# mackelab/poisson-gpfa

Measured on AMD Instinct MI355X. Metric: EM iterations/sec, higher is better.
Workload: dtype f64

## Files before the change

poisson-gpfa_amd/csrc/chol.h:

```cpp
#pragma once
#include "types.h"

namespace pgpfa {


__device__ __forceinline__ int potrf_lidx(int j, int r) { return j * NB - (j * (j - 1)) / 2 + (r - j); }

template <typename T>
struct PotrfLds {
  T L[NB * (NB + 1) / 2];
  T line[2][NB];
  T rd[2];
  T rowc[2][2][64];
  T colc[2][NB];
};

template <typename T>
__device__ __forceinline__ T pick8(const T* a, int k) {
  const T v01 = (k & 1) ? a[1] : a[0], v23 = (k & 1) ? a[3] : a[2];
  const T v45 = (k & 1) ? a[5] : a[4], v67 = (k & 1) ? a[7] : a[6];
  const T v03 = (k & 2) ? v23 : v01, v47 = (k & 2) ? v67 : v45;
  return (k & 4) ? v47 : v03;
}

template <int Q, typename T>
__device__ __forceinline__ void potrf_diag_chol_steps(T (&a)[32], PotrfLds<T>& S, int r, int cg, int pos_r,
                                                       int* __restrict__ info, long long slot, int k0) {
#pragma unroll 1
  for (int j = 32 * Q; j < 32 * Q + 32; ++j) {
    const bool own = (j & 3) == cg;
    T* buf = S.line[j & 1];
    if (own && r >= j) {
      const T v = pick8(&a[8 * Q], (j >> 2) - 8 * Q);
      buf[pos_r] = v;
      if (r == j) {
        T rd = rsqrt(v);
        if (!(v > (T)0)) {
          if (info[slot] == 0) info[slot] = k0 + j + 1;
          rd = (T)1;
        }
        S.rd[j & 1] = rd;
      }
    }
    __syncthreads();
    if (r >= j) {
      const T rd = S.rd[j & 1];
      const T lr = buf[pos_r] * rd;
      if (own) S.L[potrf_lidx(j, r)] = lr;
      const T nlr = -lr * rd;
      const T* bp = buf + cg * 32;
#pragma unroll
      for (int m = 8 * Q; m < 32; ++m) a[m] = fma(nlr, bp[m], a[m]);
    }
  }
}

template <int S, typename T>
__device__ __forceinline__ void potrf_diag_chol_steps2(T (&a)[4][8], PotrfLds<T>& L, int tr, int tc, int* __restrict__ info, long long slot, int k0) {
  typedef T v2 __attribute__((ext_vector_type(2)));
#pragma unroll 1
  for (int j = 16 * S; j < 16 * S + 16; ++j) {
    const int b = j & 1;
    if (tc == (j & 15)) {
      *reinterpret_cast<v2*>(&L.rowc[b][0][2 * tr]) = v2{a[0][S], a[1][S]};
      *reinterpret_cast<v2*>(&L.rowc[b][1][2 * tr]) = v2{a[2][S], a[3][S]};
#pragma unroll
      for (int i = 0; i < 4; ++i) L.colc[b][(tr & 15) * 8 + 2 * i + (tr >> 4)] = a[i][S];
      if (tr == (j & 31)) {
        const T v = (j >> 5) == 0 ? a[0][S] : (j >> 5) == 1 ? a[1][S] : (j >> 5) == 2 ? a[2][S] : a[3][S];
        T rd = rsqrt(v);
        if (!(v > (T)0)) {
          if (info[slot] == 0) info[slot] = k0 + j + 1;
          rd = (T)1;
        }
        L.rd[b] = rd;
      }
    }
    __syncthreads();
    const T rd = L.rd[b];
    const v2 r01 = *reinterpret_cast<const v2*>(&L.rowc[b][0][2 * tr]), r23 = *reinterpret_cast<const v2*>(&L.rowc[b][1][2 * tr]);
    T lr[4] = {r01.x * rd, r01.y * rd, r23.x * rd, r23.y * rd};
    if (tc == (j & 15)) {
#pragma unroll
      for (int i = 0; i < 4; ++i) {
        const int r = tr + 32 * i;
        if (r >= j) L.L[potrf_lidx(j, r)] = lr[i];
      }
    }
    T cv[8];
#pragma unroll
    for (int m = S & ~1; m < 8; m += 2) {
      const v2 c2 = *reinterpret_cast<const v2*>(&L.colc[b][8 * tc + m]);
      cv[m] = c2.x; cv[m + 1] = c2.y;
    }
#pragma unroll
    for (int i = 0; i < 4; ++i) {
      const T nlr = -lr[i] * rd;
#pragma unroll
      for (int m = S; m < 8; ++m) a[i][m] = fma(nlr, cv[m], a[i][m]);
    }
  }
}

template <typename T>
__device__ __forceinline__ void potrf_diag_inverse(PotrfLds<T>& S, int tid, int r, int cg) {
  const int Q = r >> 5, rl = r & 31;
  const T inv_lrr = (T)1 / S.L[potrf_lidx(r, r)];
  T t[8];
#pragma unroll
  for (int m = 0; m < 8; ++m) t[m] = (T)0;
#pragma unroll 1
  for (int il = 0; il < 32; ++il) {
    T* xrow = S.line[il & 1] + Q * 32 + cg * 8;
    if (rl == il) {
#pragma unroll
      for (int m = 0; m < 8; ++m) xrow[m] = t[m];
      if ((il & 3) == cg) xrow[il >> 2] = inv_lrr;
    }
    __syncthreads();
    if (rl > il) {
      const T lri = -S.L[potrf_lidx(32 * Q + il, r)] * inv_lrr;
#pragma unroll
      for (int m = 0; m < 8; ++m) t[m] = fma(lri, xrow[m], t[m]);
    }
  }
  __syncthreads();
#pragma unroll
  for (int m = 0; m < 8; ++m) {
    const int c = 32 * Q + cg + 4 * m;
    if (c < r) S.L[potrf_lidx(c, r)] = t[m];
  }
  if ((rl & 3) == cg) S.L[potrf_lidx(r, r)] = inv_lrr;
  __syncthreads();
  using V4 = typename GemmVec<T>::v4;
  const int lane = tid & 63, wave = tid >> 6, l15 = lane & 15, l4 = lane >> 4;
  auto lrow = [](int i) { return i * (NB - 1) - (i * (i - 1)) / 2; };
  auto xoff = [](int c) { return c * NB - (c * (c - 1)) / 2 - c; };
#pragma unroll 1
  for (int P = 1; P < 4; ++P) {
    const int ntile = 4 * P;
    V4 acc[2];
#pragma unroll
    for (int s2 = 0; s2 < 2; ++s2) {
      acc[s2] = V4{(T)0, (T)0, (T)0, (T)0};
      const int tile = wave + 8 * s2;
      if (tile < ntile) {
        const int rt = tile & 1, ct = tile >> 1;
        const int row = 32 * P + 16 * rt + l15, col = 16 * ct + l15;
        const int xo = xoff(col);
        for (int k0 = 16 * ct; k0 < 32 * P; k0 += 4) {
          const int k = k0 + l4;
          const T av = S.L[lrow(k) + row];
          const T bv = S.L[xo + k];
          acc[s2] = gemm_mfma16(av, (k >= col) ? bv : (T)0, acc[s2]);
        }
      }
    }
    __syncthreads();
#pragma unroll
    for (int s2 = 0; s2 < 2; ++s2) {
      const int tile = wave + 8 * s2;
      if (tile < ntile) {
        const int rt = tile & 1, ct = tile >> 1;
        const int xo = xoff(16 * ct + l15);
#pragma unroll
        for (int q = 0; q < 4; ++q) S.L[xo + 32 * P + 16 * rt + (sizeof(T) == 8 ? l4 + 4 * q : 4 * l4 + q)] = acc[s2][q];
      }
    }
    __syncthreads();
#pragma unroll
    for (int s2 = 0; s2 < 2; ++s2) {
      acc[s2] = V4{(T)0, (T)0, (T)0, (T)0};
      const int tile = wave + 8 * s2;
      if (tile < ntile) {
        const int rt = tile & 1, ct = tile >> 1;
        const int row = 32 * P + 16 * rt + l15;
        const int xo = xoff(16 * ct + l15);
        for (int k0 = 32 * P; k0 < 32 * P + 16 * (rt + 1); k0 += 4) {
          const int k = k0 + l4;
          const T av = S.L[lrow(k <= row ? k : row) + row];
          const T bv = S.L[xo + k];
          acc[s2] = gemm_mfma16((k <= row) ? -av : (T)0, bv, acc[s2]);
        }
      }
    }
    __syncthreads();
#pragma unroll
    for (int s2 = 0; s2 < 2; ++s2) {
      const int tile = wave + 8 * s2;
      if (tile < ntile) {
        const int rt = tile & 1, ct = tile >> 1;
        const int xo = xoff(16 * ct + l15);
#pragma unroll
        for (int q = 0; q < 4; ++q) S.L[xo + 32 * P + 16 * rt + (sizeof(T) == 8 ? l4 + 4 * q : 4 * l4 + q)] = acc[s2][q];
      }
    }
    __syncthreads();
  }
}

template <typename T, int PH = 3, int ALG = 2, typename TS = T>
__global__ __launch_bounds__(512) void potrf_diag_kernel_t(TS* __restrict__ H, long long sH, int ld, int k0,
                                                            TS* __restrict__ Dinv, long long sD,
                                                            const int* __restrict__ slots, int* __restrict__ info) {
  __shared__ __attribute__((aligned(16))) PotrfLds<T> S;
  const int tid = threadIdx.x;
  const int r = tid & (NB - 1);
  const int cg = tid >> 7;
  const int pos_r = (r & 3) * 32 + (r >> 2);
  const long long slot = slots ? slots[blockIdx.x] : blockIdx.x;
  TS* Hs = H + slot * sH + (size_t)k0 * ld + k0;
  TS* Ds = Dinv + slot * sD + (size_t)(k0 / NB) * NB * NB;

  if constexpr (ALG == 2) {
    const int tr = tid & 31, tc = tid >> 5;
    T a2[4][8];
#pragma unroll
    for (int i = 0; i < 4; ++i)
#pragma unroll
      for (int m = 0; m < 8; ++m) a2[i][m] = (T)Hs[(size_t)(tc + 16 * m) * ld + tr + 32 * i];
    if constexpr (PH & 1) {
      potrf_diag_chol_steps2<0>(a2, S, tr, tc, info, slot, k0);
      potrf_diag_chol_steps2<1>(a2, S, tr, tc, info, slot, k0);
      potrf_diag_chol_steps2<2>(a2, S, tr, tc, info, slot, k0);
      potrf_diag_chol_steps2<3>(a2, S, tr, tc, info, slot, k0);
      potrf_diag_chol_steps2<4>(a2, S, tr, tc, info, slot, k0);
      potrf_diag_chol_steps2<5>(a2, S, tr, tc, info, slot, k0);
      potrf_diag_chol_steps2<6>(a2, S, tr, tc, info, slot, k0);
      potrf_diag_chol_steps2<7>(a2, S, tr, tc, info, slot, k0);
    } else {
#pragma unroll
      for (int i = 0; i < 4; ++i)
#pragma unroll
        for (int m = 0; m < 8; ++m)
          if (tc + 16 * m <= tr + 32 * i) S.L[potrf_lidx(tc + 16 * m, tr + 32 * i)] = a2[i][m];
    }
  } else {
    T a[32];
#pragma unroll
    for (int m = 0; m < 32; ++m) a[m] = (T)Hs[(size_t)(cg + 4 * m) * ld + r];
    if constexpr (PH & 1) {
      potrf_diag_chol_steps<0>(a, S, r, cg, pos_r, info, slot, k0);
      potrf_diag_chol_steps<1>(a, S, r, cg, pos_r, info, slot, k0);
      potrf_diag_chol_steps<2>(a, S, r, cg, pos_r, info, slot, k0);
      potrf_diag_chol_steps<3>(a, S, r, cg, pos_r, info, slot, k0);
    } else {
#pragma unroll
      for (int m = 0; m < 32; ++m)
        if (cg + 4 * m <= r) S.L[potrf_lidx(cg + 4 * m, r)] = a[m];
    }
  }
  __syncthreads();
  for (int e = tid; e < NB * NB; e += 512) {
    const int rr = e & (NB - 1), cc = e >> 7;
    if (rr >= cc) Hs[(size_t)cc * ld + rr] = (TS)S.L[potrf_lidx(cc, rr)];
  }
  if constexpr (PH & 2) potrf_diag_inverse(S, tid, r, cg);
  for (int e = tid; e < NB * NB; e += 512) {
    const int rr = e & (NB - 1), cc = e >> 7;
    Ds[(size_t)cc * NB + rr] = (rr >= cc) ? (TS)S.L[potrf_lidx(cc, rr)] : (TS)0;
  }
}

template <typename T>
__global__ void diag_transpose_kernel_t(T* __restrict__ Mt, long long sM, int ld, int k0,
                                        const T* __restrict__ Dinv, long long sD, const int* __restrict__ slots) {
  const long long slot = slots ? slots[blockIdx.x] : blockIdx.x;
  k0 += blockIdx.y * NB;
  T* M = Mt + slot * sM + (size_t)k0 * ld + k0;
  const T* D = Dinv + slot * sD + (size_t)(k0 / NB) * NB * NB;
  __shared__ T tile[32][33];
  const int tx = threadIdx.x & 31, ty = threadIdx.x >> 5;
  for (int sub = 0; sub < 16; ++sub) {
    const int br = (sub & 3) * 32, bc = (sub >> 2) * 32;
    __syncthreads();
#pragma unroll
    for (int i = 0; i < 4; ++i) tile[ty + 8 * i][tx] = D[(br + ty + 8 * i) * NB + bc + tx];
    __syncthreads();
#pragma unroll
    for (int i = 0; i < 4; ++i) M[(size_t)(bc + ty + 8 * i) * ld + br + tx] = tile[tx][ty + 8 * i];
  }
}

inline __global__ __launch_bounds__(256) void chol_solve_kernel(const double* __restrict__ H, long long sH, int ld, int npad,
                                                          const double* __restrict__ Dinv, long long sD,
                                                          const double* __restrict__ G, double* __restrict__ V,
                                                          long long sV, const int* __restrict__ slots,
                                                          double* __restrict__ dec, double* __restrict__ smax, int n) {
  __shared__ double yk[NB];
  __shared__ double zk[NB];
  __shared__ double red[8];
  const int tid = threadIdx.x;
  const int lane = tid & 63, wave = tid >> 6;
  const long long slot = slots ? slots[blockIdx.x] : blockIdx.x;
  const double* L = H + slot * sH;
  const double* D = Dinv + slot * sD;
  const double* g = G + slot * sV;
  double* v = V + slot * sV;
  const int nblk = npad / NB;

  for (int i = tid; i < npad; i += 256) v[i] = (i < n) ? g[i] : 0.0;
  __syncthreads();
  for (int kb = 0; kb < nblk; ++kb) {
    const int k0 = kb * NB;
// ... 60 lines not shown
```

poisson-gpfa_amd/csrc/core.hip:

```cpp
#include "ctx.h"
#include "model.h"
#include "dual.h"
#include "thin.h"
#include "hook.h"
#include "plan.h"

using namespace pgpfa;

static_assert(plan::Dims{}.NB == NB && plan::Dims{}.WIDE_MAX == WIDE_MAX, "plan.h restates two constants of the kernel headers (workspace.hip includes none)");

thread_local std::string g_err;
thread_local unsigned long long g_fail_count = 0;

int fail(const char* fmt, ...) {
  char buf[1024];
  va_list ap;
  va_start(ap, fmt);
  vsnprintf(buf, sizeof(buf), fmt, ap);
  va_end(ap);
  g_err = buf;
  ++g_fail_count;
  return 1;
}

// ... 820 lines not shown
  };
  if (k == "newton_xtol") c->xtol = v;
  else if (k == "newton_max_iter") c->max_iter = (int)v;
  else if (k == "use_mfma") {
    const bool was = c->mfma;
    c->mfma = (v != 0.0);
    if (c->have_params && c->rank_gran != 16 && was != c->mfma)
      CHK(pgpfa_set_params(c, std::vector<double>(c->hC).data(), std::vector<double>(c->hd).data(), std::vector<double>(c->htau).data()));
  }
  else if (k == "cd_mfma") c->cd_mfma = (v != 0.0);
  else if (k == "cd_hess_mfma") c->cd_hess_mfma = (v != 0.0);
  else if (k == "cross_kernel") c->cross_kernel = (v != 0.0);
  else if (k == "cd_debug") c->cd_debug = (int)v;
  else if (k == "pcg_fused") c->pcg_fused = (int)v;
  else if (k == "pcg_w32") c->pcg_w32 = (v != 0.0);
  else if (k == "pcg_form") c->pcg_form = (int)v;
  else if (k == "pcg_vec32") c->pcg_vec32 = (int)v;
  else if (k == "pcg_rx32") c->pcg_rx32 = (int)v;
  else if (k == "pcg_adapt") c->pcg_adapt = (int)v;
  else if (k == "pcg_xcd") c->pcg_xcd = (int)v;
  else if (k == "mt_fill") c->mt_fill = (int)v;
  else if (k == "overlap_factors") c->overlap_factors = (int)v;
  else if (k == "mix_slot") c->mix_slot = (int)v;
  else if (k == "yt_mix") c->yt_mix = (v != 0.0);
  else if (k == "pivchol_pairs") c->pivchol_pairs = (v != 0.0);
  else if (k == "vsm_b4") c->vsm_b4 = (int)v;
  else if (k == "poisson_tiles") c->poisson_tiles = (int)v;
  else if (k == "yt_mix_dbg") c->yt_mix_dbg = (int)v;
  else if (k == "yt_mix_dma") c->yt_mix_dma = (v != 0.0);
  else if (k == "syrk_dbg") c->syrk_dbg = (int)v;
  else if (k == "syrk_tile") c->syrk_tile = (int)v;
  else if (k == "mix_wide") c->mix_wide = (int)v;
  else if (k == "thin_products") {
    const bool was = c->thin_products >= 2;
    c->thin_products = (int)v;
    if (c->have_params && c->rank_gran != 16 && was != (c->thin_products >= 2))
      CHK(pgpfa_set_params(c, std::vector<double>(c->hC).data(), std::vector<double>(c->hd).data(), std::vector<double>(c->htau).data()));
  }
  else if (k == "copy_kernels") c->copy_kernels = (v != 0.0);
  else if (k == "chord") c->chord = (v != 0.0);
  else if (k == "shared_pcg") c->shared_pcg = (v != 0.0);
  else if (k == "time_newton") c->time_newton = (v != 0.0);
  else if (k == "pcg_trace") c->pcg_trace = (v != 0.0);
  else if (k == "measure_mix") { c->measure_mix = (v != 0.0); c->info["last_eps_wt_norm"] = 0.0; c->info["last_eps_wt_rms"] = 0.0; }
  else if (k == "pcg_retire") c->pcg_retire = (v != 0.0);
  else if (k == "split_cov") c->split_cov = (v != 0.0);
  else if (k == "split_max_norm") c->split_max_norm = v;
  else if (k == "cov_mode") c->cov_mode = (int)v;
  else if (k == "lowrank_tol") {
    const bool changed = c->lr_tol != v;
    c->lr_tol = v;
    if (c->have_params && changed)
      CHK(pgpfa_set_params(c, std::vector<double>(c->hC).data(), std::vector<double>(c->hd).data(), std::vector<double>(c->htau).data()));
  }
  else if (k == "keep_trial_vsmgp") c->keep_trial_vsmgp = (v != 0.0);
  else if (k == "dual_lowrank") c->dual_lowrank = (v != 0.0);
  else if (k == "dual_f32") c->dual_f32 = (int)v;
  else if (k == "laplace_f32") { if (v != 0.0 && v != 1.0 && v != 2.0) return fail("laplace_f32 is 0, 1 or 2"); c->laplace_f32 = (int)v; }
  else if (k == "dual_masked") { if (v != 0.0 && v != 1.0) return fail("dual_masked is 0 or 1"); c->dual_masked = (int)v; }
  else if (k == "laplace_evidence") { if (v != 0.0 && v != 1.0) return fail("laplace_evidence is 0 or 1"); c->laplace_evidence = (int)v; }
  else if (k == "sample_chunk_trials") CHK(chunk_trials(&c->sample_chunk));
  else if (k == "interp_chunk_trials") CHK(chunk_trials(&c->interp_chunk));
  else if (k == "covat_chunk_trials") CHK(chunk_trials(&c->covat_chunk));
  else if (k == "velat_chunk_trials") CHK(chunk_trials(&c->velat_chunk));
  else if (k == "covat_block_times") { if (v < 0.0 || v != std::floor(v)) return fail("covat_block_times is a count of query times, or 0"); c->covat_block = (int)v; }
  else if (k == "func_chunk_trials") CHK(chunk_trials(&c->func_chunk));
  else if (k == "func_block_cols") {
    if (v < 0.0 || v != std::floor(v) || std::fmod(v, 16.0) != 0.0) return fail("func_block_cols is a count of functionals that is a multiple of 16, or 0");
    c->func_block = (int)v;
  }
  else if (k == "rates_chunk_trials") CHK(chunk_trials(&c->rates_chunk));
  else if (k == "counts_chunk_trials") CHK(chunk_trials(&c->counts_chunk));
  else if (k == "counts_nodes") { if (v < 8.0 || v > 64.0 || v != std::floor(v)) return fail("counts_nodes is a node count in 8 .. 64"); c->counts_Q = (int)v; }
  else if (k == "slab_row_align") c->slab_row_align = (v != 0.0);
  else if (k == "vsm_mfma") c->vsm_mfma = (v != 0.0);
  else if (k == "dual_gemm") c->dual_gemm = (v != 0.0);
  else if (k == "extrapolate_start") c->extrapolate = (v != 0.0);
  else if (k == "extrapolate_beta") c->extrapolate_beta = v;
  else if (k == "extrapolate_guard") c->extrapolate_guard = v;
  else if (k == "start_guard") c->start_guard = (v != 0.0);
  else if (k == "shared_min") c->shared_min = (int)v;
  else if (k == "pcg_inner") c->pcg_inner_max = std::max(1, (int)v);
  else if (k == "pcg_eta0") c->pcg_eta0 = v;
  else if (k == "splitk_target") c->splitk_target = std::max(1, (int)v);
  else if (k == "small_tile_below") c->small_tile_below = (int)v;
  else if (k == "f32_tile64") c->f32_tile64 = (int)v;
  else if (k == "splitk_below64") c->splitk_below64 = (int)v;
  else if (k == "pcg_outer_max") c->pcg_outer_max = (int)v;
  else if (k == "chord_xtol") c->chord_xtol = v;
  else if (k == "chord_rho") c->chord_rho = v;
  else if (k == "chord_max_step") c->chord_max_step = v;
  else if (k == "chord_max") c->chord_max = (int)v;
  else if (k == "chunk_trials") { if (c->B > 0) return fail("chunk_trials must be set before the first E-step"); c->chunk_opt = (int)v; }
  else if (k == "workspace_headroom") c->arena_headroom = std::max(1.0, v);
  else if (k == "rank_gran") { if (v != 4.0 && v != 8.0 && v != 16.0) return fail("rank_gran is 4, 8 or 16"); c->rank_gran = (int)v; if (c->have_params) CHK(pgpfa_set_params(c, std::vector<double>(c->hC).data(), std::vector<double>(c->hd).data(), std::vector<double>(c->htau).data())); }
  else if (k == "workspace_pool") { if (c->arena_cap > 0) return fail("workspace_pool must be set before the first E-step"); c->use_pool = (v != 0.0); }
  else if (k == "workspace_grow_budget_ms") c->grow_budget_ms = v;
  else if (k == "workspace_grow_floor_slots") c->grow_floor_slots = std::max(1, (int)v);
  else if (k == "workspace_granule_mb") c->vmm_granule = (size_t)std::max(2.0, v) << 20;
  else if (k == "workspace_vmm") { if (c->arena_cap > 0) return fail("workspace_vmm must be set before the first E-step"); c->vmm = (v != 0.0) ? 0 : -1; }
  else if (k == "eps_noise") {
    const bool changed = c->eps != v;
    c->eps = v;
    if (c->have_params && changed)
      CHK(pgpfa_set_params(c, std::vector<double>(c->hC).data(), std::vector<double>(c->hd).data(), std::vector<double>(c->htau).data()));
  }
  else if (k == "profile") {
    if (v != 0.0) {
      prof_collect(c);
      c->prof.ms.clear(); c->prof.flops.clear(); c->prof.count.clear(); c->prof.max_ms.clear(); c->prof.max_flops.clear(); c->prof.shapes.clear();
      HIPC(hipSetDevice(c->device));
      const size_t want = 2 * (256 + 64) + 2;
      while (c->prof.pool.size() < want) {
        hipEvent_t e;
        HIPC(hipEventCreate(&e));
        c->prof.pool.push_back(e);
        c->prof.idle.push_back(e);
      }
      for (int rep = 0; rep < 8; ++rep)
        for (hipEvent_t e : c->prof.idle) HIPC(hipEventRecord(e, c->st));
      HIPC(hipStreamSynchronize(c->st));
    }
    c->prof.on = (v != 0.0);
    c->prof.configured = c->prof.on;
    c->prof.only_tag = (v == 2.0) ? TAG_GEMM : (v == 3.0) ? TAG_MIX : -1;
  } else if (k == "profile_pause") {
    c->prof.on = (v == 0.0) && c->prof.configured;
  } else return fail("unknown option '%s'", key);
  return 0;
}

int pgpfa_get_info(pgpfa_ctx* c, const char* key, double* value) {
  if (!c || !key || !value) return fail("null argument");
  const std::string k(key);
  static const char* tags[TAG_N] = {"gemm", "potrf", "solve", "poisson", "assemble", "vsm", "cd", "mix"};
  if (k.rfind("prof_", 0) == 0) {
    prof_collect(c);
    for (int t = 0; t < TAG_N; ++t) {
      const std::string base = std::string("prof_") + tags[t];
      if (k == base + "_ms") { *value = c->prof.ms[t]; return 0; }
      if (k == base + "_flops") { *value = c->prof.flops[t]; return 0; }
      if (k == base + "_launches") { *value = c->prof.count[t]; return 0; }
      if (k == base + "_max_ms") { *value = c->prof.max_ms[t]; return 0; }
      if (k == base + "_max_flops") { *value = c->prof.max_flops[t]; return 0; }
    }
    return fail("unknown info key '%s'", key);
  }
  if (k == "sample_noise_dim") {
    if (!c->have_params) return fail("set_params has not been called");
    *value = (double)(c->n + (want_lowrank(c) ? c->rtot : 0));
    return 0;
  }
  if (k == "hbm_bytes_allocated") { *value = (double)c->bytes; return 0; }
  if (k == "hbm_bytes_free" || k == "hbm_bytes_total") {
    size_t free_b = 0, total_b = 0;
    HIPC(hipSetDevice(c->device));
    HIPC(hipMemGetInfo(&free_b, &total_b));
    *value = (double)(k == "hbm_bytes_free" ? free_b : total_b);
    return 0;
  }
  if (k == "n_trials_global") { *value = c->n_trials_global; return 0; }
  auto it = c->info.find(k);
  if (it == c->info.end()) return fail("unknown info key '%s'", key);
  *value = it->second;
  return 0;
}
// ... 484 lines not shown
```

poisson-gpfa_amd/csrc/ctx.h:

```cpp
#pragma once
#include <hip/hip_runtime.h>
#include <rccl/rccl.h>

#include <algorithm>
#include <limits>
#include <chrono>
#include <cmath>
#include <cstdarg>
#include <cstdio>
#include <cstring>
#include <deque>
#include <functional>
#include <map>
#include <string>
#include <type_traits>
#include <vector>

#include <mutex>
#include <rocprofiler-sdk-roctx/roctx.h>
#include "../../include/pgpfa.h"
#include "types.h"
#include "live.h"

namespace pgpfa { struct ThinP; }
// ... 126 lines not shown
  int B = 0;
  double grow_budget_ms = 200.0;
  int grow_floor_slots = 128;
  bool use_pool = true;
  int plan_target = 0;
  int want_slots = 0;
  bool B_capped = false;
  CholWS ws{};
  double *Xc = nullptr, *Xt = nullptr, *KX = nullptr, *KD = nullptr, *Gl = nullptr, *Glt = nullptr, *Gt = nullptr, *Dl = nullptr;
  double *W = nullptr, *Wt = nullptr, *fpart = nullptr;
  double *lamd = nullptr, *dgrad = nullptr, *dpart = nullptr, *ldet_buf = nullptr;
  double* voff = nullptr;
  bool var_active = false, lam_out_active = false;
  double* dual_scr = nullptr; long long dual_sscr = 0;
  CholWS sws{};
  double *sU = nullptr, *sDinvT = nullptr, *Wbar = nullptr;
  double *Rv = nullptr, *Zv = nullptr, *Pv = nullptr, *Qv = nullptr;
  PcgCtl* pcgctl = nullptr;
  int* live0 = nullptr; float *pcg_ratio = nullptr, *pcg_eta = nullptr;
  int* live1 = nullptr;
  int* pcg_blk = nullptr;
  const int* cur_ndev = nullptr;
  bool live_gemm_collect = false;
  std::vector<std::pair<std::string, double>> live_gemms;
  bool pcg_retire = true;
  int* h_pcg = nullptr; int* d_hpcg = nullptr;
  float* W32 = nullptr;
  double* sc_part2 = nullptr;
  int pcg_fused = 1; bool pcg_w32 = true;
  int mt_fill = 1;
  int pcg_xcd = 1;
  int pcg_adapt = 1;
  int pcg_form = 2;
  int pcg_rx32 = 1;
  int pcg_vec32 = 1;
  double *Sv = nullptr, *cg_scal = nullptr;
  double *GbT = nullptr, *WbT = nullptr;
  double *sc_rz = nullptr, *sc_pq = nullptr, *sc_rr = nullptr, *sc_rr0 = nullptr, *sc_pack = nullptr;
  double* Flr = nullptr;
  double* Gbin = nullptr;
  int *d_rank = nullptr, *d_blk_lat = nullptr, *d_blk_col = nullptr, *d_roff = nullptr;
  int *d_kr_ft = nullptr, *d_kr_f = nullptr;
  int kr_ft_len = 0, kr_f_len = 0;
  int ntab_ft = 0, ntab_f = 0; size_t tab_cap = 0;
  int *d_thin_ft = nullptr, *d_thin_f = nullptr, *d_thin_s = nullptr;
  int nthin_ft = 0, nthin_f = 0, nthin_s = 0;
  int thin_products = 2;
  double *Fbig = nullptr, *FTbig = nullptr, *Gbar = nullptr, *Wtbar = nullptr;
  std::vector<int> rk, roff;
  std::vector<int> rr, roff16;
  int rtot = 0, rpad = 0, rtot16 = 0;
  int rank_gran = 4;
  bool rank_compact = false;
  int *d_roff16 = nullptr, *d_cmap = nullptr, *d_nrtab = nullptr;
  int cov_mode = 0;
  double lr_tol = 1e-10;
  bool plan_lowrank = false;
  size_t slab_elems = 0, mt_elems = 0, ws_mark = 0;
  char* arena = nullptr; size_t arena_cap = 0, arena_off = 0; int arena_mode = 0;
  int vmm = 0; size_t va_size = 0, vmm_gran = 0, vmm_granule = (size_t)1 << 30;
  std::vector<std::pair<hipMemGenericAllocationHandle_t, size_t>> vmm_chunks;
  double arena_headroom = 2.0;
  bool mt_dirty = false;
  bool last_cov_lowrank = false;
  bool shared_pcg = true;
  bool pcg_trace = false;
  double* zero16 = nullptr;
  double* sink = nullptr;
  int mix_wide = 1;
  int poisson_tiles = 2;
  int vsm_b4 = 2;
  int pivchol_pairs = 1;
  int yt_mix = 1;
  int syrk_tile = 256;
  int syrk_dbg = 0;
  int yt_mix_dma = 1;
  int yt_mix_dbg = 0;
  int mix_slot = 3;
  bool cross_kernel = true;
  bool measure_mix = false;
  bool time_newton = false;
  int shared_min = 16, pcg_inner_min = 2, pcg_inner_max = 16, pcg_outer_max = 12;
  double pcg_eta0 = 1e-2;
  int splitk_target = 1280;
  int f32_tile64 = 1;
  int small_tile_below = 1 << 30;
  int splitk_below64 = 400;
  double *sc_f = nullptr, *sc_qxx = nullptr, *sc_qdx = nullptr, *sc_qdd = nullptr, *sc_dec = nullptr, *sc_smax = nullptr, *sc_alpha = nullptr;
  int *trial_of_slot = nullptr, *list_a = nullptr, *list_b = nullptr, *ident = nullptr;
  int* mask_of_slot = nullptr;
  bool mask_active = false;
  CholWS kws{};
  double *tK = nullptr, *tM = nullptr, *tA1 = nullptr, *tA2 = nullptr, *tscal = nullptr, *tpart = nullptr;
  double* hbuf = nullptr; size_t hbuf_len = 0;
  struct DlEntry { void* host; size_t off, bytes; };
  PcgCtl fused_ctl_host{};
  char* dl_stage = nullptr; size_t dl_used = 0; std::vector<DlEntry> dl_pending;
  char* dl_stage_dev = nullptr; char* ring_dev = nullptr;
  unsigned* h_seq = nullptr; unsigned* d_seq = nullptr; unsigned seq_next = 0;
  bool copy_kernels = true;
  unsigned long long dl_fail_mark = 0;
  int* hibuf = nullptr; size_t hibuf_len = 0;
  char* ring = nullptr; size_t ring_slot = 0; int ring_cur = 0, ring_pending = 0;
  std::map<std::string, double> info;
  std::vector<void*> allocs;
  size_t bytes = 0;
  Prof prof;
  ncclComm_t comm = nullptr;
  int rank = 0, nranks = 1;
  double* commbuf = nullptr; size_t commbuf_len = 0;
  double* rates_tbl = nullptr; double rates_tbl_params = -1.0;
  int rates_chunk = 0;
  int sample_chunk = 0;
  int interp_chunk = 0;
  int covat_chunk = 0;
  int velat_chunk = 0;
  int covat_block = 0;
  int func_chunk = 0;
  int func_block = 0;
  int counts_chunk = 0;
  int counts_Q = 32;
  double* counts_nodes = nullptr; int counts_nodes_Q = 0;
};

inline bool thin_possible(const pgpfa_ctx* c) { return c->thin_products && c->mfma && c->T >= 4; }

struct BLayout {
  int nblk64, npairs;
  const int* cmap;
  const int* roff_padded;
  const int* nrtab;
  int ncmap_rows;
};
BLayout b_layout(const pgpfa_ctx* c);
BLayout b_layout_of(bool compact, int rtot16, int rpad, const int* cmap, const int* roff_padded, const int* nrtab);
struct RankLayout {
  std::vector<int> rr, rk, roff, roff16;
  int rtot = 0, rtot16 = 0, rpad = 0;
  bool rank_compact = false;
  std::vector<int> blk_lat, blk_col;
  std::vector<int> cmap, nrtab;
  int bad_pair = -1;
};
RankLayout rank_layout(int p, const int* ranks, int gran, bool thin_all);
inline CholWS lowrank_view(const pgpfa_ctx* c, const CholWS& ws) {
  CholWS lw = ws;
  lw.ld = c->rpad; lw.npad = c->rpad; lw.nact = round_up(c->rtot, 64);
  return lw;
}

template <typename T>
int dmalloc(pgpfa_ctx* c, T** out, size_t count, bool zero = false) {
  void* p = nullptr;
  const size_t bytes = std::max<size_t>(count, 1) * sizeof(T);
  if (c->arena_mode) {
    const size_t aligned = (bytes + 255) & ~(size_t)255;
    *out = nullptr;
    if (c->arena_mode == 2) {
      if (c->arena_off + aligned > c->arena_cap) return fail("workspace arena overflow (%zu + %zu > %zu bytes)", c->arena_off, aligned, c->arena_cap);
      p = c->arena + c->arena_off;
      if (zero && hipMemsetAsync(p, 0, bytes, c->st) != hipSuccess) return fail("hipMemset failed");
      *out = reinterpret_cast<T*>(p);
    }
    c->arena_off += aligned;
    return 0;
  }
// ... 154 lines not shown
```

poisson-gpfa_amd/csrc/linalg.hip:

```cpp
#include "ctx.h"
#include "model.h"
#include "gemm.h"
#include "chol.h"

using namespace pgpfa;

double gemm_flops(const GemmP& g) {
  if (g.flops_hint > 0.0) return g.flops_hint;
  const double M = g.M, N = g.N, K = g.K;
  double per;
  if (g.mode == GEMM_LOWER) {
    const double elems = N * (M - N) + N * (N + 1) / 2.0;
    per = 2.0 * K * elems;
  } else if (g.kflags & KF_BEGIN_ROW) {
    per = 2.0 * N * (M * K - M * (M - 1) / 2.0);
  } else if (g.kflags & KF_BEGIN_MAXRC) {
    per = 0.0;
    const double m = std::min(M, N);
    per = 2.0 * (M * N * K - (m * (m - 1) * (m + 1) / 3.0 + (M > N ? N * (M - N) * (M + N - 1) / 2.0 : M * (N - M) * (M + N - 1) / 2.0)));
  } else {
    per = 2.0 * M * N * K;
  }
  return per * g.nbatch;
}

int gemm(pgpfa_ctx* c, bool transb, GemmP g, bool f32) {
  const bool live_cols = g.cols && c->cur_ndev;
  prof_begin(c, TAG_GEMM, live_cols ? 0.0 : gemm_flops(g));
  if (c->prof.on && c->prof.open) {
    char key[176];
    std::snprintf(key, sizeof key, "%s %s M=%d N=%s%d K=%d%s batch=%d%s%s%s", f32 ? "f32" : "f64", transb ? "NN" : "NT", g.M, live_cols ? "<=" : "", g.N,
                  g.K, g.kseg ? " (segmented)" : "", std::max(g.nbatch, 1), g.mode == GEMM_LOWER ? " lower" : "",
                  g.kflags ? " triangular-k" : "", g.rtab ? " block-sparse" : "");
    c->prof.recs.back().shape = key;
    if (live_cols && c->live_gemm_collect) c->live_gemms.emplace_back(key, gemm_flops(g) / std::max(g.N, 1));
  }
  if (g.bm == 0) {
    const long long t128 = (long long)((g.M + GBM - 1) / GBM) * ((g.N + GBN - 1) / GBN) * std::max(g.nbatch, 1);
    g.bm = ((!f32 || c->f32_tile64) && c->mfma && (g.rtab || t128 < c->small_tile_below)) ? 64 : 128;
  }
  if (g.rtab) g.bm = 64;
  if (g.cols && c->cur_ndev) g.n_dev = c->cur_ndev;
  if ((const double*)g.C == g.A || (const double*)g.C == g.B) g.bm = 128;
  const int tiles = (g.rtab ? g.ntab : (g.M + g.bm - 1) / g.bm) * ((g.N + g.bm - 1) / g.bm) * std::max(g.nbatch, 1);
  int ksplit = 1;
  const double k_eff = g.k_loop_hint > 0 ? (double)g.k_loop_hint
                       : (g.flops_hint > 0.0 && g.M > 0 && g.N > 0) ? g.flops_hint / (2.0 * g.M * g.N * std::max(g.nbatch, 1)) : (double)g.K;
  const int split_below = g.bm == 64 ? c->splitk_below64 : 384;
  if (!f32 && c->gemm_part && !c->no_splitk && g.mode == GEMM_FULL && g.kflags == 0 && g.nb_lo == 0 && g.kseg == 0 && tiles > 0 && tiles < split_below && k_eff >= 128.0) {
    ksplit = std::min(std::min(8, (int)(k_eff / (tiles < 64 ? 32.0 : 64.0))), (c->splitk_target + tiles - 1) / tiles);
    while (ksplit > 1 && (size_t)ksplit * g.nbatch * g.M * g.N > c->gemm_part_len) --ksplit;
  }
  hipError_t e;
  if (ksplit > 1) {
    GemmP s = g;
    s.C = c->gemm_part; s.sC = (long long)g.M * g.N; s.ldc = g.M; s.beta = 0.0;
    s.nb_lo = g.nbatch; s.nbatch = g.nbatch * ksplit; s.sA_hi = 0; s.sB_hi = 0; s.sC_hi = (long long)g.nbatch * g.M * g.N;
    s.ksplit = ksplit;
    s.c_by_pos = 1;
    s.cols_c_off = 1;
    e = gemm_launch(c->st, c->mfma, transb, s);
    if (e == hipSuccess) {
      hipLaunchKernelGGL(gemm_splitk_reduce_kernel, dim3((unsigned)(((size_t)g.M * g.N + 255) / 256), g.nbatch), dim3(256), 0, c->st, c->gemm_part,
                         ksplit, g.M, g.N, g.nbatch, g.C, g.sC, g.ldc, g.slots, g.beta, g.skip, g.cols, g.n_dev);
      e = hipGetLastError();
    }
  } else {
    e = gemm_launch(c->st, c->mfma, transb, g, f32);
  }
  prof_end(c);
  if (e != hipSuccess) return fail("gemm launch failed: %s", hipGetErrorString(e));
  return 0;
}

int factor(pgpfa_ctx* c, const CholWS& w, const int* slots, int nb, bool f32, bool wide_diag) {
  auto at = [f32](double* base, size_t off) { return f32 ? reinterpret_cast<double*>(reinterpret_cast<float*>(base) + off) : base + off; };
  const int np = w.npad, ld = w.ld;
  const int na = (w.nact > 0 && w.nact <= np) ? w.nact : np;
  for (int c0 = 0; c0 < np; c0 += NSUP) {
    const int c1 = std::min(c0 + NSUP, np);
    for (int k0 = c0; k0 < c1; k0 += NB) {
      prof_begin(c, TAG_POTRF, 2.0 * nb * (double)NB * NB * NB / 3.0);
      if (f32 && wide_diag)
        hipLaunchKernelGGL((potrf_diag_kernel_t<double, 3, 2, float>), dim3(nb), dim3(512), 0, c->st, reinterpret_cast<float*>(w.H), w.sH, ld, k0,
                           reinterpret_cast<float*>(w.Dinv), w.sD, slots, w.info);
      else if (f32)
        hipLaunchKernelGGL(potrf_diag_kernel_t<float>, dim3(nb), dim3(512), 0, c->st, reinterpret_cast<float*>(w.H), w.sH, ld, k0,
                           reinterpret_cast<float*>(w.Dinv), w.sD, slots, w.info);
      else
        hipLaunchKernelGGL(potrf_diag_kernel_t<double>, dim3(nb), dim3(512), 0, c->st, w.H, w.sH, ld, k0, w.Dinv, w.sD, slots, w.info);
      prof_end(c);
      const int r0 = k0 + NB;
      if (r0 >= np) break;
      GemmP g{};
      g.A = at(w.H, (size_t)k0 * ld + r0); g.sA = w.sH; g.lda = ld;
      g.B = at(w.Dinv, (size_t)(k0 / NB) * NB * NB); g.sB = w.sD; g.ldb = NB;
      g.C = at(w.H, (size_t)k0 * ld + r0); g.sC = w.sH; g.ldc = ld;
      g.M = na - r0; g.N = NB; g.K = NB; g.alpha = 1.0; g.beta = 0.0;
      g.slots = slots; g.nbatch = nb; g.mode = GEMM_FULL; g.kflags = 0;
      if (g.M > 0) CHK(gemm(c, false, g, f32));
      if (r0 < c1 && r0 < na) {
        GemmP s{};
        s.A = at(w.H, (size_t)k0 * ld + r0); s.sA = w.sH; s.lda = ld;
        s.B = s.A; s.sB = w.sH; s.ldb = ld;
        s.C = at(w.H, (size_t)r0 * ld + r0); s.sC = w.sH; s.ldc = ld;
        s.M = na - r0; s.N = std::min(c1, na) - r0; s.K = NB; s.alpha = -1.0; s.beta = 1.0;
        s.slots = slots; s.nbatch = nb; s.mode = GEMM_LOWER; s.kflags = KF_MASK_DIAG;
        CHK(gemm(c, false, s, f32));
      }
    }
    if (c1 < na) {
      GemmP s{};
      s.A = at(w.H, (size_t)c0 * ld + c1); s.sA = w.sH; s.lda = ld;
      s.B = s.A; s.sB = w.sH; s.ldb = ld;
      s.C = at(w.H, (size_t)c1 * ld + c1); s.sC = w.sH; s.ldc = ld;
      s.M = na - c1; s.N = na - c1; s.K = c1 - c0; s.alpha = -1.0; s.beta = 1.0;
      s.slots = slots; s.nbatch = nb; s.mode = GEMM_LOWER; s.kflags = KF_MASK_DIAG;
      CHK(gemm(c, false, s, f32));
    }
  }
  HIPC(hipGetLastError());
  return 0;
}

int inverse_t(pgpfa_ctx* c, const CholWS& w, const int* slots, int nb, bool f32) {
  auto at = [f32](double* base, size_t off) { return f32 ? reinterpret_cast<double*>(reinterpret_cast<float*>(base) + off) : base + off; };
  const int np = w.npad, ld = w.ld;
  const int na = (w.nact > 0 && w.nact <= np) ? w.nact : np;
  if (f32)
    hipLaunchKernelGGL(diag_transpose_kernel_t<float>, dim3(nb, np / NB), dim3(256), 0, c->st, reinterpret_cast<float*>(w.Mt), w.sM, ld, 0,
                       reinterpret_cast<const float*>(w.Dinv), w.sD, slots);
  else
    hipLaunchKernelGGL(diag_transpose_kernel_t<double>, dim3(nb, np / NB), dim3(256), 0, c->st, w.Mt, w.sM, ld, 0, w.Dinv, w.sD, slots);
  for (int j0 = NB; j0 < np; j0 += NB) {
    const int nbw = std::min(NB, na - j0);
    if (nbw <= 0) continue;
    GemmP a{};
    a.A = w.Mt; a.sA = w.sM; a.lda = ld;
    a.B = at(w.H, j0); a.sB = w.sH; a.ldb = ld;
    a.C = w.P; a.sC = w.sP; a.ldc = np;
    a.M = std::min(j0, na); a.N = nbw; a.K = j0; a.alpha = 1.0; a.beta = 0.0;
    a.slots = slots; a.nbatch = nb; a.mode = GEMM_FULL; a.kflags = KF_BEGIN_ROW;
    CHK(gemm(c, false, a, f32));
    GemmP b{};
    b.A = w.P; b.sA = w.sP; b.lda = np;
    b.B = at(w.Dinv, (size_t)(j0 / NB) * NB * NB); b.sB = w.sD; b.ldb = NB;
    b.C = at(w.Mt, (size_t)j0 * ld); b.sC = w.sM; b.ldc = ld;
    b.M = std::min(j0, na); b.N = nbw; b.K = nbw; b.alpha = -1.0; b.beta = 0.0;
    b.slots = slots; b.nbatch = nb; b.mode = GEMM_FULL; b.kflags = 0;
    CHK(gemm(c, false, b, f32));
  }
  HIPC(hipGetLastError());
  return 0;
}


int pgpfa_test_potrf(pgpfa_ctx* c, int batch, int n, const double* A, double* L, double* inv) {
  if (!c || !A || !L) return fail("null argument");
  if (batch < 1 || n < 1) return fail("invalid sizes");
  HIPC(hipSetDevice(c->device));
  const int np = round_up(n, NB);
  CholWS w{};
  const size_t mark = c->allocs.size();
  CHK(alloc_cholws(c, &w, batch, np, true));
  const size_t slab = (size_t)np * np;
  std::vector<double> h(slab * batch, 0.0);
  for (int b = 0; b < batch; ++b) {
    double* s = h.data() + slab * b;
    for (int j = 0; j < np; ++j)
      for (int i = 0; i < np; ++i) s[(size_t)j * np + i] = (i < n && j < n) ? A[((size_t)b * n + i) * n + j] : (i == j ? 1.0 : 0.0);
  }
  int rc = upload(c, w.H, h.data(), slab * batch);
  if (!rc) rc = factor(c, w, nullptr, batch);
// ... 98 lines not shown
  return test_gemm(c, false, M, N, K, alpha, A, B, beta, C);
}
int pgpfa_test_gemm_nn(pgpfa_ctx* c, int M, int N, int K, double alpha, const double* A, const double* B, double beta, double* C) {
  return test_gemm(c, true, M, N, K, alpha, A, B, beta, C);
}

int pgpfa_bench_mfma_peak(pgpfa_ctx* c, int iters, double* tflops) {
  if (!c || !tflops || iters < 1) return fail("invalid argument");
  HIPC(hipSetDevice(c->device));
  const int blocks = 256 * 8;
  double* out = nullptr;
  HIPC(hipMalloc((void**)&out, (size_t)blocks * 256 * sizeof(double)));
  hipEvent_t e0, e1;
  hipEventCreate(&e0); hipEventCreate(&e1);
  hipLaunchKernelGGL(mfma_peak_kernel, dim3(blocks), dim3(256), 0, c->st, out, iters);
  hipEventRecord(e0, c->st);
  hipLaunchKernelGGL(mfma_peak_kernel, dim3(blocks), dim3(256), 0, c->st, out, iters);
  hipEventRecord(e1, c->st);
  hipEventSynchronize(e1);
  float ms = 0.f;
  hipEventElapsedTime(&ms, e0, e1);
  hipEventDestroy(e0); hipEventDestroy(e1);
  hipFree(out);
  HIPC(hipGetLastError());
  const double flops = (double)blocks * 4.0 * iters * 8.0 * 2048.0;
  *tflops = flops / (ms * 1e-3) / 1e12;
  return 0;
}

int pgpfa_bench_syrk(pgpfa_ctx* c, int batch, int n, int k, int reps, double* ms_per_launch, double* flops_per_launch) {
  if (!c || !ms_per_launch || !flops_per_launch) return fail("null argument");
  if (n % 128 != 0 || k % 16 != 0 || batch < 1 || reps < 1) return fail("n must be a multiple of 128 and k of 16");
  HIPC(hipSetDevice(c->device));
  const size_t mark = c->allocs.size();
  double *dC = nullptr, *dA = nullptr;
  CHK(dmalloc(c, &dC, (size_t)n * n * batch));
  CHK(dmalloc(c, &dA, (size_t)n * k * batch));
  hipLaunchKernelGGL(fill_kernel, dim3((unsigned)(((size_t)n * n * batch + 255) / 256)), dim3(256), 0, c->st, dC, (size_t)n * n * batch, 1.0);
  hipLaunchKernelGGL(fill_kernel, dim3((unsigned)(((size_t)n * k * batch + 255) / 256)), dim3(256), 0, c->st, dA, (size_t)n * k * batch, 1e-3);
  GemmP s{};
  s.A = dA; s.sA = (long long)n * k; s.lda = n; s.B = dA; s.sB = s.sA; s.ldb = n;
  s.C = dC; s.sC = (long long)n * n; s.ldc = n; s.M = n; s.N = n; s.K = k; s.alpha = -1e-6; s.beta = 1.0;
  s.nbatch = batch; s.mode = GEMM_LOWER; s.kflags = KF_MASK_DIAG;
  hipEvent_t e0, e1;
  hipEventCreate(&e0); hipEventCreate(&e1);
  int rc = 0;
  for (int i = 0; i < 2 && !rc; ++i) rc = gemm_launch(c->st, c->mfma, false, s) != hipSuccess;
  hipEventRecord(e0, c->st);
  for (int i = 0; i < reps && !rc; ++i) rc = gemm_launch(c->st, c->mfma, false, s) != hipSuccess;
  hipEventRecord(e1, c->st);
  hipEventSynchronize(e1);
  float ms = 0.f;
  hipEventElapsedTime(&ms, e0, e1);
  hipEventDestroy(e0); hipEventDestroy(e1);
  *ms_per_launch = ms / reps;
  *flops_per_launch = gemm_flops(s);
  while (c->allocs.size() > mark) { hipFree(c->allocs.back()); c->allocs.pop_back(); }
  if (rc) return fail("syrk bench launch failed");
  return 0;
}

int pgpfa_gemm_shape_report(pgpfa_ctx* c, char* buf, int len) {
  if (!c || (len > 0 && !buf)) { fail("null argument"); return -1; }
  prof_collect(c);
  std::vector<std::pair<std::string, Prof::Shape>> v(c->prof.shapes.begin(), c->prof.shapes.end());
  std::sort(v.begin(), v.end(), [](const auto& a, const auto& b) { return a.second.ms > b.second.ms; });
  std::string out;
  char line[256];
  for (const auto& kv : v) {
    std::snprintf(line, sizeof line, "%-74s n=%6.0f  %9.2f ms  %10.1f GFLOP  %6.1f TFLOP/s\n", kv.first.c_str(), kv.second.count, kv.second.ms,
                  kv.second.flops * 1e-9, kv.second.ms > 0.0 ? kv.second.flops / kv.second.ms * 1e-9 : 0.0);
    out += line;
  }
  if (len > 0) {
    const size_t n = std::min(out.size(), (size_t)len - 1);
    std::memcpy(buf, out.data(), n);
    buf[n] = 0;
  }
  return (int)out.size() + 1;
}

int pgpfa_bench_potrf_diag(pgpfa_ctx* c, int batch, int reps, int phases, double* us_per_launch) {
  if (!c || !us_per_launch) return fail("null argument");
  if (batch < 1 || reps < 1 || (phases != 0 && phases != 1 && phases != 3 && phases != 5 && phases != 7)) return fail("batch, reps >= 1; phases 0, 1 or 3 (+ 4: the round-1 form of the Cholesky steps)");
  HIPC(hipSetDevice(c->device));
  const size_t mark = c->allocs.size();
  double *dH = nullptr, *dD = nullptr;
  int* dinfo = nullptr;
  const size_t blk = (size_t)NB * NB;
  CHK(dmalloc(c, &dH, blk * batch));
  CHK(dmalloc(c, &dD, blk * batch));
  CHK(dmalloc(c, &dinfo, (size_t)batch, true));
  std::vector<double> h(blk);
  for (int j = 0; j < NB; ++j)
    for (int i = 0; i < NB; ++i) h[(size_t)j * NB + i] = (i == j ? 2.0 : 0.0) + 1.0 / (1.0 + std::abs(i - j));
  for (int b = 0; b < batch; ++b) HIPC(hipMemcpyAsync(dH + blk * b, h.data(), blk * sizeof(double), hipMemcpyHostToDevice, c->st));
  HIPC(hipStreamSynchronize(c->st));
  hipEvent_t e0, e1;
  hipEventCreate(&e0); hipEventCreate(&e1);
  auto launch = [&]() {
    if (phases == 7)
      hipLaunchKernelGGL((potrf_diag_kernel_t<double, 3, 1>), dim3(batch), dim3(512), 0, c->st, dH, (long long)blk, NB, 0, dD, (long long)blk, (const int*)nullptr, dinfo);
    else if (phases == 5)
      hipLaunchKernelGGL((potrf_diag_kernel_t<double, 1, 1>), dim3(batch), dim3(512), 0, c->st, dH, (long long)blk, NB, 0, dD, (long long)blk, (const int*)nullptr, dinfo);
    else if (phases == 3)
      hipLaunchKernelGGL((potrf_diag_kernel_t<double, 3>), dim3(batch), dim3(512), 0, c->st, dH, (long long)blk, NB, 0, dD, (long long)blk, (const int*)nullptr, dinfo);
    else if (phases == 1)
      hipLaunchKernelGGL((potrf_diag_kernel_t<double, 1>), dim3(batch), dim3(512), 0, c->st, dH, (long long)blk, NB, 0, dD, (long long)blk, (const int*)nullptr, dinfo);
    else
      hipLaunchKernelGGL((potrf_diag_kernel_t<double, 0>), dim3(batch), dim3(512), 0, c->st, dH, (long long)blk, NB, 0, dD, (long long)blk, (const int*)nullptr, dinfo);
  };
  launch();
  hipEventRecord(e0, c->st);
  for (int i = 0; i < reps; ++i) launch();
  hipEventRecord(e1, c->st);
  hipEventSynchronize(e1);
  float ms = 0.f;
  hipEventElapsedTime(&ms, e0, e1);
  hipEventDestroy(e0); hipEventDestroy(e1);
  *us_per_launch = 1e3 * ms / reps;
  while (c->allocs.size() > mark) { hipFree(c->allocs.back()); c->allocs.pop_back(); }
  HIPC(hipGetLastError());
  return 0;
}
```

Baseline: 12.42.

## Factor diagonal Cholesky block in panels of four columns per barrier

Adds a panel variant of the in-block Cholesky steps. A 4-wide panel of columns is staged in LDS, each row thread factors it redundantly, and the trailing update is applied as a rank-4 update. This cuts the number of __syncthreads rounds per diagonal block by about four times, and the new variant is on by default through a potrf_panel context option. It also pins waves_per_eu to 4 on the kernel. The cost is redundant small factorizations per thread and a larger LDS footprint.

Measured after the change: 12.52 (median of 6 runs). About the same (+0.8%).

```diff
diff --git a/poisson-gpfa_amd/csrc/chol.h b/poisson-gpfa_amd/csrc/chol.h
--- a/poisson-gpfa_amd/csrc/chol.h
+++ b/poisson-gpfa_amd/csrc/chol.h
@@ -6,7 +6,7 @@
 
 __device__ __forceinline__ int potrf_lidx(int j, int r) { return j * NB - (j * (j - 1)) / 2 + (r - j); }
 
-template <typename T>
+template <typename T, int PW = 1>
 struct PotrfLds {
   T L[NB * (NB + 1) / 2];
   T line[2][NB];
@@ -14,6 +14,14 @@
   T rowc[2][2][64];
   T colc[2][NB];
 };
+template <typename T>
+struct PotrfLds<T, 4> {
+  T L[NB * (NB + 1) / 2];
+  T line[2][NB];
+  T rd[2];
+  T raw[NB * 4], tx[NB * 4], tnl[NB * 4];
+};
+__device__ __forceinline__ int potrf_pidx(int c, int t) { return (t >> 1) * (2 * NB) + 2 * c + (t & 1); }
 
 template <typename T>
 __device__ __forceinline__ T pick8(const T* a, int k) {
@@ -23,8 +31,8 @@
   return (k & 4) ? v47 : v03;
 }
 
-template <int Q, typename T>
-__device__ __forceinline__ void potrf_diag_chol_steps(T (&a)[32], PotrfLds<T>& S, int r, int cg, int pos_r,
+template <int Q, typename T, int PW>
+__device__ __forceinline__ void potrf_diag_chol_steps(T (&a)[32], PotrfLds<T, PW>& S, int r, int cg, int pos_r,
                                                        int* __restrict__ info, long long slot, int k0) {
 #pragma unroll 1
   for (int j = 32 * Q; j < 32 * Q + 32; ++j) {
@@ -55,8 +63,8 @@
   }
 }
 
-template <int S, typename T>
-__device__ __forceinline__ void potrf_diag_chol_steps2(T (&a)[4][8], PotrfLds<T>& L, int tr, int tc, int* __restrict__ info, long long slot, int k0) {
+template <int S, typename T, int PW>
+__device__ __forceinline__ void potrf_diag_chol_steps2(T (&a)[4][8], PotrfLds<T, PW>& L, int tr, int tc, int* __restrict__ info, long long slot, int k0) {
   typedef T v2 __attribute__((ext_vector_type(2)));
 #pragma unroll 1
   for (int j = 16 * S; j < 16 * S + 16; ++j) {
@@ -102,8 +110,92 @@
   }
 }
 
-template <typename T>
-__device__ __forceinline__ void potrf_diag_inverse(PotrfLds<T>& S, int tid, int r, int cg) {
+template <int S, int W, typename T, int PW>
+__device__ __forceinline__ void potrf_diag_chol_steps3(T (&a)[4][8], PotrfLds<T, PW>& L, int tid, int tr, int tc, int* __restrict__ info, long long slot, int k0) {
+  typedef T v2 __attribute__((ext_vector_type(2)));
+  static_assert((W == 2 || W == 4) && W <= PW, "a panel lies inside one group of 16 columns and is read in 16-byte pieces");
+#pragma unroll 1
+  for (int j = 16 * S; j < 16 * S + 16; j += W) {
+    const int t_own = tc - (j & 15);
+    if ((unsigned)t_own < (unsigned)W) {
+#pragma unroll
+      for (int i = 0; i < 4; ++i) L.raw[potrf_pidx(tr + 32 * i, t_own)] = a[i][S];
+    }
+    __syncthreads();
+    if (tid < NB && tid >= j) {
+      const int c = tid;
+      T pv[W][W], rd[W], x[W], nl[W];
+#pragma unroll
+      for (int u = 0; u < W; ++u)
+#pragma unroll
+        for (int h = 0; h < W; h += 2) {
+          const v2 x2 = *reinterpret_cast<const v2*>(&L.raw[potrf_pidx(j + u, h)]);
+          pv[u][h] = x2.x; pv[u][h + 1] = x2.y;
+        }
+#pragma unroll
+      for (int h = 0; h < W; h += 2) {
+        const v2 x2 = *reinterpret_cast<const v2*>(&L.raw[potrf_pidx(c, h)]);
+        x[h] = x2.x; x[h + 1] = x2.y;
+      }
+#pragma unroll
+      for (int s = 0; s < W; ++s) {
+        const T v = pv[s][s];
+        T r1 = rsqrt(v);
+        if (!(v > (T)0)) {
+          if (c == j && info[slot] == 0) info[slot] = k0 + j + s + 1;
+          r1 = (T)1;
+        }
+        rd[s] = r1;
+#pragma unroll
+        for (int u = s + 1; u < W; ++u) {
+          const T lr = pv[u][s] * r1;
+          const T nlr = -lr * r1;
+#pragma unroll
+          for (int u2 = s + 1; u2 <= u; ++u2) pv[u][u2] = fma(nlr, pv[u2][s], pv[u][u2]);
+        }
+      }
+#pragma unroll
+      for (int s = 0; s < W; ++s) {
+        const T lr = x[s] * rd[s];
+        if (c >= j + s) L.L[potrf_lidx(j + s, c)] = lr;
+        const T nlr = -lr * rd[s];
+        nl[s] = nlr;
+#pragma unroll
+        for (int u = s + 1; u < W; ++u) x[u] = fma(nlr, pv[u][s], x[u]);
+      }
+#pragma unroll
+      for (int h = 0; h < W; h += 2) {
+        *reinterpret_cast<v2*>(&L.tx[potrf_pidx(c, h)]) = v2{x[h], x[h + 1]};
+        *reinterpret_cast<v2*>(&L.tnl[potrf_pidx(c, h)]) = v2{nl[h], nl[h + 1]};
+      }
+    }
+    __syncthreads();
+    T nl[4][W];
+#pragma unroll
+    for (int i = 0; i < 4; ++i)
+#pragma unroll
+      for (int h = 0; h < W; h += 2) {
+        const v2 x2 = *reinterpret_cast<const v2*>(&L.tnl[potrf_pidx(tr + 32 * i, h)]);
+        nl[i][h] = x2.x; nl[i][h + 1] = x2.y;
+      }
+#pragma unroll
+    for (int m = S; m < 8; ++m) {
+      T x[W];
+#pragma unroll
+      for (int h = 0; h < W; h += 2) {
+        const v2 x2 = *reinterpret_cast<const v2*>(&L.tx[potrf_pidx(tc + 16 * m, h)]);
+        x[h] = x2.x; x[h + 1] = x2.y;
+      }
+#pragma unroll
+      for (int i = 0; i < 4; ++i)
+#pragma unroll
+        for (int s = 0; s < W; ++s) a[i][m] = fma(nl[i][s], x[s], a[i][m]);
+    }
+  }
+}
+
+template <typename T, int PW>
+__device__ __forceinline__ void potrf_diag_inverse(PotrfLds<T, PW>& S, int tid, int r, int cg) {
   const int Q = r >> 5, rl = r & 31;
   const T inv_lrr = (T)1 / S.L[potrf_lidx(r, r)];
   T t[8];
@@ -199,11 +291,11 @@
   }
 }
 
-template <typename T, int PH = 3, int ALG = 2, typename TS = T>
-__global__ __launch_bounds__(512) void potrf_diag_kernel_t(TS* __restrict__ H, long long sH, int ld, int k0,
+template <typename T, int PH = 3, int ALG = 2, typename TS = T, int W = 4>
+__global__ __launch_bounds__(512) __attribute__((amdgpu_waves_per_eu(4, 4))) void potrf_diag_kernel_t(TS* __restrict__ H, long long sH, int ld, int k0,
                                                             TS* __restrict__ Dinv, long long sD,
                                                             const int* __restrict__ slots, int* __restrict__ info) {
-  __shared__ __attribute__((aligned(16))) PotrfLds<T> S;
+  __shared__ __attribute__((aligned(16))) PotrfLds<T, (ALG == 3 ? 4 : 1)> S;
   const int tid = threadIdx.x;
   const int r = tid & (NB - 1);
   const int cg = tid >> 7;
@@ -212,14 +304,23 @@
   TS* Hs = H + slot * sH + (size_t)k0 * ld + k0;
   TS* Ds = Dinv + slot * sD + (size_t)(k0 / NB) * NB * NB;
 
-  if constexpr (ALG == 2) {
+  if constexpr (ALG == 2 || ALG == 3) {
     const int tr = tid & 31, tc = tid >> 5;
     T a2[4][8];
 #pragma unroll
     for (int i = 0; i < 4; ++i)
 #pragma unroll
       for (int m = 0; m < 8; ++m) a2[i][m] = (T)Hs[(size_t)(tc + 16 * m) * ld + tr + 32 * i];
-    if constexpr (PH & 1) {
+    if constexpr ((PH & 1) && ALG == 3) {
+      potrf_diag_chol_steps3<0, W>(a2, S, tid, tr, tc, info, slot, k0);
+      potrf_diag_chol_steps3<1, W>(a2, S, tid, tr, tc, info, slot, k0);
+      potrf_diag_chol_steps3<2, W>(a2, S, tid, tr, tc, info, slot, k0);
+      potrf_diag_chol_steps3<3, W>(a2, S, tid, tr, tc, info, slot, k0);
+      potrf_diag_chol_steps3<4, W>(a2, S, tid, tr, tc, info, slot, k0);
+      potrf_diag_chol_steps3<5, W>(a2, S, tid, tr, tc, info, slot, k0);
+      potrf_diag_chol_steps3<6, W>(a2, S, tid, tr, tc, info, slot, k0);
+      potrf_diag_chol_steps3<7, W>(a2, S, tid, tr, tc, info, slot, k0);
+    } else if constexpr (PH & 1) {
       potrf_diag_chol_steps2<0>(a2, S, tr, tc, info, slot, k0);
       potrf_diag_chol_steps2<1>(a2, S, tr, tc, info, slot, k0);
       potrf_diag_chol_steps2<2>(a2, S, tr, tc, info, slot, k0);
diff --git a/poisson-gpfa_amd/csrc/core.hip b/poisson-gpfa_amd/csrc/core.hip
--- a/poisson-gpfa_amd/csrc/core.hip
+++ b/poisson-gpfa_amd/csrc/core.hip
@@ -926,6 +926,7 @@
   else if (k == "shared_min") c->shared_min = (int)v;
   else if (k == "pcg_inner") c->pcg_inner_max = std::max(1, (int)v);
   else if (k == "pcg_eta0") c->pcg_eta0 = v;
+  else if (k == "potrf_panel") { if (v != 1.0 && v != 4.0) return fail("potrf_panel is 1 or 4"); c->potrf_panel = (int)v; }
   else if (k == "splitk_target") c->splitk_target = std::max(1, (int)v);
   else if (k == "small_tile_below") c->small_tile_below = (int)v;
   else if (k == "f32_tile64") c->f32_tile64 = (int)v;
diff --git a/poisson-gpfa_amd/csrc/ctx.h b/poisson-gpfa_amd/csrc/ctx.h
--- a/poisson-gpfa_amd/csrc/ctx.h
+++ b/poisson-gpfa_amd/csrc/ctx.h
@@ -232,6 +232,7 @@
   bool time_newton = false;
   int shared_min = 16, pcg_inner_min = 2, pcg_inner_max = 16, pcg_outer_max = 12;
   double pcg_eta0 = 1e-2;
+  int potrf_panel = 4;
   int splitk_target = 1280;
   int f32_tile64 = 1;
   int small_tile_below = 1 << 30;
diff --git a/poisson-gpfa_amd/csrc/linalg.hip b/poisson-gpfa_amd/csrc/linalg.hip
--- a/poisson-gpfa_amd/csrc/linalg.hip
+++ b/poisson-gpfa_amd/csrc/linalg.hip
@@ -81,14 +81,17 @@
     const int c1 = std::min(c0 + NSUP, np);
     for (int k0 = c0; k0 < c1; k0 += NB) {
       prof_begin(c, TAG_POTRF, 2.0 * nb * (double)NB * NB * NB / 3.0);
-      if (f32 && wide_diag)
-        hipLaunchKernelGGL((potrf_diag_kernel_t<double, 3, 2, float>), dim3(nb), dim3(512), 0, c->st, reinterpret_cast<float*>(w.H), w.sH, ld, k0,
-                           reinterpret_cast<float*>(w.Dinv), w.sD, slots, w.info);
-      else if (f32)
-        hipLaunchKernelGGL(potrf_diag_kernel_t<float>, dim3(nb), dim3(512), 0, c->st, reinterpret_cast<float*>(w.H), w.sH, ld, k0,
-                           reinterpret_cast<float*>(w.Dinv), w.sD, slots, w.info);
-      else
-        hipLaunchKernelGGL(potrf_diag_kernel_t<double>, dim3(nb), dim3(512), 0, c->st, w.H, w.sH, ld, k0, w.Dinv, w.sD, slots, w.info);
+      const bool panel = c->potrf_panel > 1;
+      if (f32 && wide_diag) {
+        auto* k = panel ? potrf_diag_kernel_t<double, 3, 3, float> : potrf_diag_kernel_t<double, 3, 2, float>;
+        hipLaunchKernelGGL(k, dim3(nb), dim3(512), 0, c->st, reinterpret_cast<float*>(w.H), w.sH, ld, k0, reinterpret_cast<float*>(w.Dinv), w.sD, slots, w.info);
+      } else if (f32) {
+        auto* k = panel ? potrf_diag_kernel_t<float, 3, 3> : potrf_diag_kernel_t<float>;
+        hipLaunchKernelGGL(k, dim3(nb), dim3(512), 0, c->st, reinterpret_cast<float*>(w.H), w.sH, ld, k0, reinterpret_cast<float*>(w.Dinv), w.sD, slots, w.info);
+      } else {
+        auto* k = panel ? potrf_diag_kernel_t<double, 3, 3> : potrf_diag_kernel_t<double>;
+        hipLaunchKernelGGL(k, dim3(nb), dim3(512), 0, c->st, w.H, w.sH, ld, k0, w.Dinv, w.sD, slots, w.info);
+      }
       prof_end(c);
       const int r0 = k0 + NB;
       if (r0 >= np) break;
@@ -353,7 +356,8 @@
 
 int pgpfa_bench_potrf_diag(pgpfa_ctx* c, int batch, int reps, int phases, double* us_per_launch) {
   if (!c || !us_per_launch) return fail("null argument");
-  if (batch < 1 || reps < 1 || (phases != 0 && phases != 1 && phases != 3 && phases != 5 && phases != 7)) return fail("batch, reps >= 1; phases 0, 1 or 3 (+ 4: the round-1 form of the Cholesky steps)");
+  if (batch < 1 || reps < 1 || (phases != 0 && phases != 1 && phases != 3 && phases != 5 && phases != 7 && phases != 9 && phases != 11))
+    return fail("batch, reps >= 1; phases 0, 1 or 3 (+ 4: the round-1 form of the Cholesky steps, + 8: the round-5 form)");
   HIPC(hipSetDevice(c->device));
   const size_t mark = c->allocs.size();
   double *dH = nullptr, *dD = nullptr;
@@ -370,14 +374,18 @@
   hipEvent_t e0, e1;
   hipEventCreate(&e0); hipEventCreate(&e1);
   auto launch = [&]() {
-    if (phases == 7)
+    if (phases == 11)
+      hipLaunchKernelGGL((potrf_diag_kernel_t<double, 3, 2>), dim3(batch), dim3(512), 0, c->st, dH, (long long)blk, NB, 0, dD, (long long)blk, (const int*)nullptr, dinfo);
+    else if (phases == 9)
+      hipLaunchKernelGGL((potrf_diag_kernel_t<double, 1, 2>), dim3(batch), dim3(512), 0, c->st, dH, (long long)blk, NB, 0, dD, (long long)blk, (const int*)nullptr, dinfo);
+    else if (phases == 7)
       hipLaunchKernelGGL((potrf_diag_kernel_t<double, 3, 1>), dim3(batch), dim3(512), 0, c->st, dH, (long long)blk, NB, 0, dD, (long long)blk, (const int*)nullptr, dinfo);
     else if (phases == 5)
       hipLaunchKernelGGL((potrf_diag_kernel_t<double, 1, 1>), dim3(batch), dim3(512), 0, c->st, dH, (long long)blk, NB, 0, dD, (long long)blk, (const int*)nullptr, dinfo);
     else if (phases == 3)
-      hipLaunchKernelGGL((potrf_diag_kernel_t<double, 3>), dim3(batch), dim3(512), 0, c->st, dH, (long long)blk, NB, 0, dD, (long long)blk, (const int*)nullptr, dinfo);
+      hipLaunchKernelGGL((potrf_diag_kernel_t<double, 3, 3>), dim3(batch), dim3(512), 0, c->st, dH, (long long)blk, NB, 0, dD, (long long)blk, (const int*)nullptr, dinfo);
     else if (phases == 1)
-      hipLaunchKernelGGL((potrf_diag_kernel_t<double, 1>), dim3(batch), dim3(512), 0, c->st, dH, (long long)blk, NB, 0, dD, (long long)blk, (const int*)nullptr, dinfo);
+      hipLaunchKernelGGL((potrf_diag_kernel_t<double, 1, 3>), dim3(batch), dim3(512), 0, c->st, dH, (long long)blk, NB, 0, dD, (long long)blk, (const int*)nullptr, dinfo);
     else
       hipLaunchKernelGGL((potrf_diag_kernel_t<double, 0>), dim3(batch), dim3(512), 0, c->st, dH, (long long)blk, NB, 0, dD, (long long)blk, (const int*)nullptr, dinfo);
   };
```
